# lukashermann/hulc

Measured on AMD Instinct MI355X. Metric: trajectory-windows/sec (seq_len=32, bs=64/GPU), higher is better.
Workload: dtype bf16; 1 GPU; HULC training step, vision goal only (use_clip_auxiliary_loss=false), B=64 windows/GPU, seq_len=32, 200x200 static + 84x84 gripper fp32 NCHW frames, fwd+loss+bwd+Adam, dropout 0.1; global_batch=64, seq_len=32, parallelism=dp1

## Files before the change

### hulc_amd/csrc/engine.h

```cpp
#pragma once
#include <algorithm>
#include <map>
#include <string>
#include <vector>

#include "iengine.h"
#include "gemm.h"
#include "kernels.h"
#include "conv_wgrad.h"
#include "conv_tile.h"
#include "conv_reg.h"
#include "tr_fused.h"
#include "rnn_persist.h"
#include "enc_tail.h"
#include "rollout_step.h"

namespace HULC_NS {

static inline int cdiv(long long a, long long b) { return (int)((a + b - 1) / b); }
#define HIP_CHECK_VOID(x) do { hipError_t e_ = (x); if (e_ != hipSuccess) { hulc_set_error("%s:%d %s", __FILE__, __LINE__, hipGetErrorString(e_)); } } while (0)

template <typename T>
struct Engine : IEngine {
    hulc_config cfg;
// ... 819 lines not shown
    }

    int optim(const hulc_optim& o) override {
        if (!bound) { hulc_set_error("hulc_optimizer_step before hulc_bind_params"); return 1; }
        const bool want_norm = clip_algo == HULC_CLIP_NORM || clip_track;
        if (want_norm && !gn_built) { hulc_set_error("hulc_optimizer_step: the gradient-norm tables are missing (hulc_bind_params / hulc_grad_clip_set build them)"); return 1; }
        persist_check("hulc_optimizer_step", false);
        lazy_sweep(0, numel, st);
        bwd_since_opt = false;
        const unsigned tag = ++opt_seq;
        if (o.kind != HULC_OPT_ADAM && o.kind != HULC_OPT_ADAMW && o.kind != HULC_OPT_SGD) { hulc_set_error("hulc_optimizer_step: unknown optimizer kind %d", (int)o.kind); return 1; }
        if (o.step < 1) { hulc_set_error("hulc_optimizer_step: step counts from 1 (got %lld)", (long long)o.step); return 1; }
        const float lr = o.lr, b1 = o.beta1, b2 = o.beta2, eps = o.eps, gscale = o.grad_scale;
        const int64_t step = o.step;
        const double bc1d = 1.0 - pow((double)b1, (double)step), bc2d = 1.0 - pow((double)b2, (double)step);
        h16_t* const shadow = std::is_same<T, float>::value ? (h16_t*)nullptr : (h16_t*)wshadow;
        const ClipState* const cs = clip_algo != HULC_CLIP_OFF ? clip_state : nullptr;
        if (want_norm) {
            hipLaunchKernelGGL(grad_sumsq_kernel, dim3(gn_chunks), dim3(256), 0, st, (const float*)G, (const long long*)gn_chunk_start, (const int*)gn_chunk_n, gn_partial, scaler);
            hipLaunchKernelGGL(grad_norm_combine_kernel, dim3(1), dim3(1024), 0, st, (const float*)gn_partial, (const int*)gn_tfirst, (int)gn_tens.size(), gscale, (const ScalerState*)scaler,
                               clip_state, gn_tsq, gn_tnorm);
            gn_have = true;
        } else if (scaler) hipLaunchKernelGGL(nonfinite_check_kernel, dim3(2048), dim3(256), 0, st, G, (long long)numel, scaler);
        if (o.kind == HULC_OPT_SGD)
            hipLaunchKernelGGL(sgd_kernel, dim3(2048), dim3(256), 0, st, P, G, AM, (long long)numel, lr, o.momentum, o.dampening, o.weight_decay, (int)(o.nesterov != 0),
                               (int)(step == 1), gscale, shadow, (const ScalerState*)scaler, (const unsigned*)rp_skip, tag, cs);
        else if (adam_fuse_tr && tr_adam.n && shadow) {
            AdamArgs a{P, G, AM, AV, lr, b1, b2, eps, (float)bc1d, (float)sqrt(bc2d), gscale, o.weight_decay, (int)(o.kind == HULC_OPT_ADAMW), shadow, (const ScalerState*)scaler, (const unsigned*)rp_skip, tag, cs};
            hipLaunchKernelGGL(adam_tiled_kernel, dim3(tr_adam.blocks + adam_chunks), dim3(256), 0, st, a, (const TrDesc*)tr_adam.desc, (const unsigned short*)tr_adam.b2d, tr_adam.blocks,
                               (const long long*)adam_chunk_start, (const int*)adam_chunk_n);
            tr_fresh = true;
        } else
            hipLaunchKernelGGL(adam_kernel, dim3(2048), dim3(256), 0, st, P, G, AM, AV, (long long)numel, lr, b1, b2, eps, (float)bc1d, (float)sqrt(bc2d), gscale,
                               shadow, (const ScalerState*)scaler, o.weight_decay, (int)(o.kind == HULC_OPT_ADAMW), (const unsigned*)rp_skip, tag, cs);
        if (scaler) hipLaunchKernelGGL(scaler_update_kernel, dim3(1), dim3(1), 0, st, scaler, (const unsigned*)rp_skip, tag);
        if (hipGetLastError() != hipSuccess) { hulc_set_error("adam launch failed"); return 1; }
        return prepare_weights(true);
    }

    int get_tensor(const char* name, float* out, int64_t cap, int64_t* n) override {
        auto it = named.find(name);
        if (it == named.end()) { hulc_set_error("hulc_get_tensor: unknown tensor '%s'", name); return 1; }
        const Named& t = it->second;
        int64_t cnt = std::min<int64_t>(cap, t.n);
        *n = cnt;
        HIP_CHECK(hipStreamSynchronize(st));
        if (t.kind == 0) { HIP_CHECK(hipMemcpy(out, t.p, cnt * sizeof(float), hipMemcpyDeviceToHost)); }
        else if (t.kind == 1) {
            std::vector<T> tmp(cnt);
            HIP_CHECK(hipMemcpy(tmp.data(), t.p, cnt * sizeof(T), hipMemcpyDeviceToHost));
            for (int64_t i = 0; i < cnt; ++i) out[i] = host_to_f(tmp[i]);
        } else {
            std::vector<int> tmp(cnt);
            HIP_CHECK(hipMemcpy(tmp.data(), t.p, cnt * sizeof(int), hipMemcpyDeviceToHost));
            for (int64_t i = 0; i < cnt; ++i) out[i] = (float)tmp[i];
        }
        return 0;
    }
    static float host_to_f(float x) { return x; }
#ifdef HULC_HALF_F16
    static float host_to_f(h16_t x) {
        const uint32_t sgn = (uint32_t)(x >> 15) << 31, ex = (x >> 10) & 31, man = x & 1023;
        uint32_t u;
        if (ex == 0) { float f = ldexpf((float)man, -24); memcpy(&u, &f, 4); u |= sgn; }
        else if (ex == 31) u = sgn | 0x7f800000u | (man << 13);
        else u = sgn | ((ex + 112) << 23) | (man << 13);
        float f; memcpy(&f, &u, 4); return f;
    }
#else
    static float host_to_f(h16_t x) { uint32_t u = ((uint32_t)x) << 16; float f; memcpy(&f, &u, 4); return f; }
#endif
    int get_plan_idx(int32_t* out, int64_t cap) override {
        HIP_CHECK(hipStreamSynchronize(st));
        int64_t cnt = std::min<int64_t>(cap, (int64_t)cur.B * NCAT);
        HIP_CHECK(hipMemcpy(out, pidx, cnt * sizeof(int), hipMemcpyDeviceToHost));
        return 0;
    }
};

int k_gemm_nt(int is_f32, const void* A, const void* B, float* C, int M, int N, int K, long long lda, long long ldb, long long ldc, const float* bias, int relu,
              void* stream) {
    hipStream_t st = (hipStream_t)stream;
    EpiP ep; ep.out = C; ep.out_f32 = 1; ep.bias = bias; ep.relu = relu & 1;
    if (!is_f32 && !(relu & 4) && M >= 512 && N >= 128) {
        const DenseLoader<h16_t> a = dense<h16_t>((const h16_t*)A, M, lda), b = dense<h16_t>((const h16_t*)B, N, ldb);
        if (gemm_glds_ok(a, b, ep, M, N, K)) {
            launch_gemm_glds(st, a, b, dense_out(ldc), ep, M, N, K);
            if (hipGetLastError() != hipSuccess) { hulc_set_error("hulc_k_gemm_nt: launch failed"); return 1; }
            return 0;
        }
    }
    if (is_f32) {
#ifdef HULC_HALF_F16
        hulc_set_error("hulc_k_gemm_nt: the fp32 kernels live in the bf16 translation unit"); return 1;
#else
        if (M >= 512 && N >= 128) launch_gemm<float, 128, 128>(st, dense<float>((const float*)A, M, lda), dense<float>((const float*)B, N, ldb), dense_out(ldc), ep, M, N, K);
        else launch_gemm<float, 64, 64>(st, dense<float>((const float*)A, M, lda), dense<float>((const float*)B, N, ldb), dense_out(ldc), ep, M, N, K);
#endif
    } else {
        if (M >= 512 && N >= 128) launch_gemm<h16_t, 128, 128>(st, dense<h16_t>((const h16_t*)A, M, lda), dense<h16_t>((const h16_t*)B, N, ldb), dense_out(ldc), ep, M, N, K);
        else launch_gemm<h16_t, 64, 64>(st, dense<h16_t>((const h16_t*)A, M, lda), dense<h16_t>((const h16_t*)B, N, ldb), dense_out(ldc), ep, M, N, K);
    }
    if (hipGetLastError() != hipSuccess) { hulc_set_error("hulc_k_gemm_nt: launch failed"); return 1; }
    return 0;
}

IEngine* make_engine(const hulc_config& cfg, int* rc) {
#ifdef HULC_HALF_F16
    auto* e = new Engine<h16_t>(cfg); *rc = e->alloc_all(); return e;
#else
    if (cfg.dtype == HULC_DTYPE_F32) { auto* e = new Engine<float>(cfg); *rc = e->alloc_all(); return e; }
    auto* e = new Engine<h16_t>(cfg); *rc = e->alloc_all(); return e;
#endif
}

}
```

### hulc_amd/csrc/gemm.h

```cpp
#pragma once
#include "common.h"

namespace HULC_NS {

struct EpiP {
    void* out = nullptr;
    int out_f32 = 0;
    int accumulate = 0;
    int atomic = 0;
    long long z_stride = 0;
    const float* bias = nullptr;
    const float* bias2 = nullptr;
    const void* res = nullptr;
    int res_f32 = 0;
    long long res_ld = 0;
    int res_rowmod = 0;
    int res_late = 0;
    const void* mask = nullptr;
    int mask_tanh = 0;
    int relu = 0;
    float alpha = 1.f;
    float drop_p = 0.f;
    unsigned long long drop_seed = 0;
    void* out2 = nullptr;
// ... 489 lines not shown
        for (int j = 0; j < TN; ++j) acc[i][j] = f32x4{0.f, 0.f, 0.f, 0.f};

    const int wm = wave >> 1, wn = wave & 1;
    if (kbeg < kend) fetch_all(kbeg);
    for (int k = kbeg; k < kend; k += BK) {
#pragma unroll
        for (int i = 0; i < APT; ++i) {
            const int q = tid + i * 256;
            if (q < BM * PPR) tile_commit<T, BM, AL::TRANSPOSED, BK>(As, ra[i], q);
        }
#pragma unroll
        for (int i = 0; i < BPT; ++i) {
            const int q = tid + i * 256;
            if (q < BN * PPR) tile_commit<T, BN, BL::TRANSPOSED, BK>(Bs, rb[i], q);
        }
        __syncthreads();
        if (k + BK < kend) fetch_all(k + BK);
        if constexpr (sizeof(T) == 2) {
            const T* ap = As + (wm * WM + (lane & 15)) * LD + (lane >> 4) * 8;
            const T* bp = Bs + (wn * WN + (lane & 15)) * LD + (lane >> 4) * 8;
#pragma unroll
            for (int kk = 0; kk < BK / 32; ++kk) {
                h16x8_t a[TM], b[TN];
#pragma unroll
                for (int i = 0; i < TM; ++i) a[i] = *reinterpret_cast<const h16x8_t*>(ap + i * 16 * LD + kk * 32);
#pragma unroll
                for (int j = 0; j < TN; ++j) b[j] = *reinterpret_cast<const h16x8_t*>(bp + j * 16 * LD + kk * 32);
#pragma unroll
                for (int i = 0; i < TM; ++i)
#pragma unroll
                    for (int j = 0; j < TN; ++j)
                        acc[i][j] = MFMA_16x16x32_H(b[j], a[i], acc[i][j], 0, 0, 0);
            }
        } else {
            const T* ap = As + (wm * WM + (lane & 15)) * LD + (lane >> 4);
            const T* bp = Bs + (wn * WN + (lane & 15)) * LD + (lane >> 4);
#pragma unroll
            for (int kk = 0; kk < BK / 4; ++kk) {
                float a[TM], b[TN];
#pragma unroll
                for (int i = 0; i < TM; ++i) a[i] = ap[i * 16 * LD + kk * 4];
#pragma unroll
                for (int j = 0; j < TN; ++j) b[j] = bp[j * 16 * LD + kk * 4];
#pragma unroll
                for (int i = 0; i < TM; ++i)
#pragma unroll
                    for (int j = 0; j < TN; ++j)
                        acc[i][j] = __builtin_amdgcn_mfma_f32_16x16x4f32(b[j], a[i], acc[i][j], 0, 0, 0);
            }
        }
        __syncthreads();
    }

    if (tid < BM) rowoff[tid] = (m0 + tid < M) ? om.offset(m0 + tid, zc) : 0;
    __syncthreads();
#pragma unroll
    for (int i = 0; i < TM; ++i) {
        const int row = m0 + wm * WM + i * 16 + (lane & 15);
        if (row < M) {
            const long long obase = rowoff[row - m0] + (long long)zs * ep.z_stride;
            const int rrow = ep.res_rowmod > 0 ? row % ep.res_rowmod : row;
#pragma unroll
            for (int j = 0; j < TN; ++j) {
                const int col = n0 + wn * WN + j * 16 + (lane >> 4) * 4;
                if (col < N) {
                    const float v4[4] = {acc[i][j][0], acc[i][j][1], acc[i][j][2], acc[i][j][3]};
                    epi_store4<T>(ep, v4, rrow, col, N, obase + col);
                }
            }
        }
    }
}

template <typename T, int BM, int BN, typename AL, typename BL, typename OM, int BK = 32>
static inline void launch_gemm(hipStream_t st, const AL& al, const BL& bl, const OM& om, const EpiP& ep, int Mmax, int N,
                               int K, int nclass = 1, int nsplit = 1) {
    if (Mmax <= 0 || N <= 0) return;
    int ksplit = K;
    if (nsplit > 1) ksplit = ((K + nsplit - 1) / nsplit + BK - 1) / BK * BK;
    dim3 grid((Mmax + BM - 1) / BM, (N + BN - 1) / BN, nclass * nsplit);
    hipLaunchKernelGGL((gemm_kernel<T, BM, BN, AL, BL, OM, BK>), grid, dim3(256), 0, st, al, bl, om, ep, N, K, nsplit, ksplit);
}

template <int NST, int NW>
DEVI void gemm_glds_body(const DenseLoader<h16_t>& al, const DenseLoader<h16_t>& bl, const DenseOut& om, const EpiP& ep, int M, int N, int K, int tiles_m, int tiles_n, int bid) {
    constexpr int STAGE = 32 * 1024;
    constexpr int PW = 16 / NW;
    constexpr int TM = 8 / NW * 2 * 2 / 2;
    constexpr int WROWS = TM * 16;
    extern __shared__ __attribute__((aligned(16))) char gg_smem[];
    typedef __attribute__((address_space(3))) char lchar;
    lchar* lds = (lchar*)gg_smem;
    const int tid = threadIdx.x, lane = tid & 63, wave = tid >> 6;
    const int g = lane >> 4, li = lane & 15;
    int tm, tn;
    {
        const int nt = tiles_m * tiles_n, per = nt / 8, rem = nt % 8;
        const int x = bid % 8, q = bid / 8;
        const int tile = x * per + min(x, rem) + q;
        constexpr int GM = 4;
        const int gsz = GM * tiles_n, grp = tile / gsz, first_m = grp * GM, gm = min(GM, tiles_m - first_m);
        tm = first_m + (tile % gsz) % gm;
        tn = (tile % gsz) / gm;
    }
    const int m0 = tm * 128, n0 = tn * 128;
    const int r = lane >> 3, cs = (lane & 7) ^ (r & 6);
    const h16_t* asrc[PW];
    const h16_t* bsrc[PW];
#pragma unroll
    for (int j = 0; j < PW; ++j) {
        asrc[j] = al.row(min(m0 + (wave * PW + j) * 8 + r, M - 1), 0).base + cs * 8;
        bsrc[j] = bl.row(min(n0 + (wave * PW + j) * 8 + r, N - 1), 0).base + cs * 8;
    }
    const int nk = (K + 63) >> 6;
    const bool khalf = (K & 63) != 0;
    auto issue = [&](int kt, int buf) {
        lchar* st = lds + buf * STAGE + wave * PW * 1024;
        long long ko = (long long)kt * 64;
        if (khalf && kt == nk - 1 && cs >= 4) ko -= 32;
#pragma unroll
        for (int j = 0; j < PW; ++j) {
            lds_dma16(asrc[j] + ko, (unsigned)(size_t)(st + j * 1024));
            lds_dma16(bsrc[j] + ko, (unsigned)(size_t)(st + 16384 + j * 1024));
        }
    };
    f32x4 acc[TM][4];
#pragma unroll
    for (int i = 0; i < TM; ++i)
#pragma unroll
        for (int j = 0; j < 4; ++j) acc[i][j] = f32x4{0.f, 0.f, 0.f, 0.f};
    const int wm = wave >> 1, wn = wave & 1;
    const int foff = (li >> 3) * 1024 + (li & 7) * 128;
#pragma unroll
    for (int j = 0; j < NST - 1; ++j)
        if (j < nk) issue(j, j);
    int buf = 0;
#pragma unroll 1
    for (int kt = 0; kt < nk; ++kt) {
        const int ahead = min(NST - 2, nk - 1 - kt);
        if constexpr (PW == 4) {
            if (ahead >= 3) asm volatile("s_waitcnt vmcnt(24)\n\ts_barrier" ::: "memory");
            else if (ahead == 2) asm volatile("s_waitcnt vmcnt(16)\n\ts_barrier" ::: "memory");
            else if (ahead == 1) asm volatile("s_waitcnt vmcnt(8)\n\ts_barrier" ::: "memory");
            else asm volatile("s_waitcnt vmcnt(0)\n\ts_barrier" ::: "memory");
        } else {
            if (ahead >= 3) asm volatile("s_waitcnt vmcnt(12)\n\ts_barrier" ::: "memory");
            else if (ahead == 2) asm volatile("s_waitcnt vmcnt(8)\n\ts_barrier" ::: "memory");
            else if (ahead == 1) asm volatile("s_waitcnt vmcnt(4)\n\ts_barrier" ::: "memory");
            else asm volatile("s_waitcnt vmcnt(0)\n\ts_barrier" ::: "memory");
        }
        if (kt + NST - 1 < nk) issue(kt + NST - 1, buf == 0 ? NST - 1 : buf - 1);
        lchar* sa = lds + buf * STAGE + wm * (WROWS / 8) * 1024 + foff;
        lchar* sb = lds + buf * STAGE + 16384 + wn * 8192 + foff;
        const int nkk = (khalf && kt == nk - 1) ? 1 : 2;
#pragma unroll 1
        for (int kk = 0; kk < nkk; ++kk) {
            const int chunk = (((kk << 2) + g) ^ (li & 6)) << 4;
            h16x8_t a[TM], b[4];
#pragma unroll
            for (int i = 0; i < TM; ++i) a[i] = *(__attribute__((address_space(3))) h16x8_t*)(sa + i * 2048 + chunk);
#pragma unroll
            for (int j = 0; j < 4; ++j) b[j] = *(__attribute__((address_space(3))) h16x8_t*)(sb + j * 2048 + chunk);
#pragma unroll
            for (int i = 0; i < TM; ++i)
#pragma unroll
                for (int j = 0; j < 4; ++j) acc[i][j] = MFMA_16x16x32_H(b[j], a[i], acc[i][j], 0, 0, 0);
        }
        buf = buf == NST - 1 ? 0 : buf + 1;
    }
    const bool plain = epi_is_plain_f32(ep) && (om.s1 & 3) == 0 && (om.s0 & 3) == 0 && ((uintptr_t)ep.out & 15) == 0;
    const bool fast16 = epi_is_fast16(ep) && (om.s1 & 3) == 0 && (om.s0 & 3) == 0;
#pragma unroll
    for (int i = 0; i < TM; ++i) {
        const int row = m0 + wm * WROWS + i * 16 + li;
        if (row < M) {
            const long long obase = om.offset(row, 0);
            const int rrow = ep.res_rowmod > 0 ? row % ep.res_rowmod : row;
#pragma unroll
            for (int j = 0; j < 4; ++j) {
                const int col = n0 + wn * 64 + j * 16 + g * 4;
                if (col < N) {
                    if (plain && col + 3 < N) { epi_plain4(ep, acc[i][j], obase + col); continue; }
                    if (fast16 && col + 3 < N) { epi_fast16_4(ep, acc[i][j], rrow, col, obase + col); continue; }
                    const float v4[4] = {acc[i][j][0], acc[i][j][1], acc[i][j][2], acc[i][j][3]};
                    epi_store4<h16_t>(ep, v4, rrow, col, N, obase + col);
                }
            }
        }
    }
}
template <int NST, int NW>
__global__ void __launch_bounds__(NW * 64) gemm_glds_kernel(DenseLoader<h16_t> al, DenseLoader<h16_t> bl, DenseOut om, EpiP ep, int M, int N, int K,
                                                           int tiles_m, int tiles_n) {
    gemm_glds_body<NST, NW>(al, bl, om, ep, M, N, K, tiles_m, tiles_n, (int)blockIdx.x);
}
struct GemmGroupP { DenseLoader<h16_t> a[3], b[3]; DenseOut om[3]; EpiP ep[3]; int M[3], N[3], K[3], tm[3], tn[3], t0[3]; int n; };
template <int NST, int NW>
__global__ void __launch_bounds__(NW * 64) gemm_glds_group_kernel(GemmGroupP g) {
    const int b = (int)blockIdx.x;
    const int p = (g.n > 2 && b >= g.t0[2]) ? 2 : ((g.n > 1 && b >= g.t0[1]) ? 1 : 0);
    const int bid = b - g.t0[p];
    if (bid >= g.tm[p] * g.tn[p]) return;
    gemm_glds_body<NST, NW>(g.a[p], g.b[p], g.om[p], g.ep[p], g.M[p], g.N[p], g.K[p], g.tm[p], g.tn[p], bid);
}
__global__ void __launch_bounds__(512) gemm_glds_pair_kernel(DenseLoader<h16_t> al, DenseLoader<h16_t> bl1, DenseLoader<h16_t> bl2, DenseOut om, EpiP ep1, EpiP ep2,
                                                           int M, int N, int K, int shs, int tiles_m, int tiles_n) {
    constexpr int NST = 3, NW = 8, STAGE = 48 * 1024, PW = 2, TM = 2, WROWS = 32;
    extern __shared__ __attribute__((aligned(16))) char gg_smem[];
    typedef __attribute__((address_space(3))) char lchar;
    lchar* lds = (lchar*)gg_smem;
    const int tid = threadIdx.x, lane = tid & 63, wave = tid >> 6;
    const int g = lane >> 4, li = lane & 15;
    int tm, tn;
    {
        const int nt = tiles_m * tiles_n, per = nt / 8, rem = nt % 8;
        const int x = blockIdx.x % 8, q = blockIdx.x / 8;
        const int tile = x * per + min(x, rem) + q;
        constexpr int GM = 4;
        const int gsz = GM * tiles_n, grp = tile / gsz, first_m = grp * GM, gm = min(GM, tiles_m - first_m);
        tm = first_m + (tile % gsz) % gm;
        tn = (tile % gsz) / gm;
    }
    const int m0 = tm * 128, n0 = tn * 128;
    const int r = lane >> 3, cs = (lane & 7) ^ (r & 6);
    const h16_t* asrc[PW];
    const h16_t* b1src[PW];
    const h16_t* b2src[PW];
#pragma unroll
    for (int j = 0; j < PW; ++j) {
        asrc[j] = al.row(min(m0 + (wave * PW + j) * 8 + r, M - 1), 0).base + cs * 8;
        b1src[j] = bl1.row(min(n0 + (wave * PW + j) * 8 + r, N - 1), 0).base + cs * 8;
        b2src[j] = bl2.row(min(n0 + (wave * PW + j) * 8 + r, N - 1), 0).base + cs * 8;
    }
    const int nk = K >> 6;
    auto issue = [&](int kt, int buf) {
        lchar* st = lds + buf * STAGE + wave * PW * 1024;
        const long long ko = (long long)kt * 64, ko1 = (long long)max(kt - shs, 0) * 64;
#pragma unroll
        for (int j = 0; j < PW; ++j) {
            lds_dma16(asrc[j] + ko, (unsigned)(size_t)(st + j * 1024));
            lds_dma16(b1src[j] + ko1, (unsigned)(size_t)(st + 16384 + j * 1024));
            lds_dma16(b2src[j] + ko, (unsigned)(size_t)(st + 32768 + j * 1024));
        }
    };
    f32x4 acc1[TM][4], acc2[TM][4];
#pragma unroll
    for (int i = 0; i < TM; ++i)
#pragma unroll
        for (int j = 0; j < 4; ++j) { acc1[i][j] = f32x4{0.f, 0.f, 0.f, 0.f}; acc2[i][j] = f32x4{0.f, 0.f, 0.f, 0.f}; }
    const int wm = wave >> 1, wn = wave & 1;
    const int foff = (li >> 3) * 1024 + (li & 7) * 128;
#pragma unroll
    for (int j = 0; j < NST - 1; ++j)
        if (j < nk) issue(j, j);
    int buf = 0;
#pragma unroll 1
    for (int kt = 0; kt < nk; ++kt) {
        const int ahead = min(NST - 2, nk - 1 - kt);
        if (ahead >= 1) asm volatile("s_waitcnt vmcnt(6)\n\ts_barrier" ::: "memory");
        else asm volatile("s_waitcnt vmcnt(0)\n\ts_barrier" ::: "memory");
        if (kt + NST - 1 < nk) issue(kt + NST - 1, buf == 0 ? NST - 1 : buf - 1);
        lchar* sa = lds + buf * STAGE + wm * (WROWS / 8) * 1024 + foff;
        lchar* sb1 = lds + buf * STAGE + 16384 + wn * 8192 + foff;
        lchar* sb2 = lds + buf * STAGE + 32768 + wn * 8192 + foff;
        const bool with1 = kt >= shs;
#pragma unroll 1
        for (int kk = 0; kk < 2; ++kk) {
            const int chunk = (((kk << 2) + g) ^ (li & 6)) << 4;
            h16x8_t a[TM], b[4], c[4];
#pragma unroll
            for (int i = 0; i < TM; ++i) a[i] = *(__attribute__((address_space(3))) h16x8_t*)(sa + i * 2048 + chunk);
#pragma unroll
            for (int j = 0; j < 4; ++j) b[j] = *(__attribute__((address_space(3))) h16x8_t*)(sb2 + j * 2048 + chunk);
#pragma unroll
            for (int j = 0; j < 4; ++j) c[j] = *(__attribute__((address_space(3))) h16x8_t*)(sb1 + j * 2048 + chunk);
#pragma unroll
            for (int i = 0; i < TM; ++i)
#pragma unroll
                for (int j = 0; j < 4; ++j) acc2[i][j] = MFMA_16x16x32_H(b[j], a[i], acc2[i][j], 0, 0, 0);
            if (with1) {
#pragma unroll
                for (int i = 0; i < TM; ++i)
#pragma unroll
                    for (int j = 0; j < 4; ++j) acc1[i][j] = MFMA_16x16x32_H(c[j], a[i], acc1[i][j], 0, 0, 0);
            }
        }
        buf = buf == NST - 1 ? 0 : buf + 1;
    }
#pragma unroll
    for (int i = 0; i < TM; ++i) {
        const int row = m0 + wm * WROWS + i * 16 + li;
        if (row < M) {
            const long long obase = om.offset(row, 0);
#pragma unroll
            for (int j = 0; j < 4; ++j) {
                const int col = n0 + wn * 64 + j * 16 + g * 4;
                if (col < N) {
                    if (((om.s1 | om.s0) & 3) == 0 && col + 3 < N) { epi_plain4(ep1, acc1[i][j], obase + col); epi_plain4(ep2, acc2[i][j], obase + col); continue; }
                    const float v1[4] = {acc1[i][j][0], acc1[i][j][1], acc1[i][j][2], acc1[i][j][3]};
                    epi_store4<h16_t>(ep1, v1, row, col, N, obase + col);
                    const float v2[4] = {acc2[i][j][0], acc2[i][j][1], acc2[i][j][2], acc2[i][j][3]};
                    epi_store4<h16_t>(ep2, v2, row, col, N, obase + col);
                }
            }
        }
    }
}
static inline bool gemm_glds_pair_ok(const DenseLoader<h16_t>& a, const DenseLoader<h16_t>& b1, const DenseLoader<h16_t>& b2, const EpiP& ep1, const EpiP& ep2, int M, int N, int K, int sh) {
    auto row_ok = [](const DenseLoader<h16_t>& l) { return (l.s0 % 8) == 0 && (l.s1 % 8) == 0 && ((uintptr_t)l.p % 16) == 0 && l.R1 == 0x7fffffff; };
    auto plain = [](const EpiP& e) {
        return !e.generic_only && e.out_f32 && !e.atomic && e.z_stride == 0 && !e.bias && !e.bias2 && !e.res && !e.mask && !e.relu && e.drop_p == 0.f && !e.out2 && e.alpha == 1.f && ((uintptr_t)e.out & 15) == 0;
    };
    return K >= 192 && (K % 64) == 0 && sh > 0 && (sh % 64) == 0 && sh < K && (M % 128) == 0 && (N % 128) == 0 && row_ok(a) && row_ok(b1) && row_ok(b2) && plain(ep1) && plain(ep2);
}
static inline void launch_gemm_glds_pair(hipStream_t st, const DenseLoader<h16_t>& a, const DenseLoader<h16_t>& b1, const DenseLoader<h16_t>& b2, const DenseOut& om, const EpiP& ep1,
                                         const EpiP& ep2, int M, int N, int K, int sh) {
    static bool attr_set = false;
    if (!attr_set) { hipFuncSetAttribute((const void*)gemm_glds_pair_kernel, hipFuncAttributeMaxDynamicSharedMemorySize, 144 * 1024); attr_set = true; }
    const int tiles_m = M / 128, tiles_n = N / 128;
    hipLaunchKernelGGL(gemm_glds_pair_kernel, dim3(tiles_m * tiles_n), dim3(512), 144 * 1024, st, a, b1, b2, om, ep1, ep2, M, N, K, sh / 64, tiles_m, tiles_n);
}
static inline bool gemm_glds_ok(const DenseLoader<h16_t>& a, const DenseLoader<h16_t>& b, const EpiP& ep, int M, int N, int K) {
    auto row_ok = [](const DenseLoader<h16_t>& l) { return (l.s0 % 8) == 0 && (l.s1 % 8) == 0 && ((uintptr_t)l.p % 16) == 0; };
    return K >= 64 && (K % 32) == 0 && ep.z_stride == 0 && row_ok(a) && row_ok(b);
}
static inline void launch_gemm_glds(hipStream_t st, const DenseLoader<h16_t>& a, const DenseLoader<h16_t>& b, const DenseOut& om, const EpiP& ep, int M, int N, int K) {
    static bool attr_set = false;
    if (!attr_set) { hipFuncSetAttribute((const void*)gemm_glds_kernel<3, 8>, hipFuncAttributeMaxDynamicSharedMemorySize, 96 * 1024); attr_set = true; }
    const int tiles_m = (M + 127) / 128, tiles_n = (N + 127) / 128;
    hipLaunchKernelGGL((gemm_glds_kernel<3, 8>), dim3(tiles_m * tiles_n), dim3(512), 96 * 1024, st, a, b, om, ep, M, N, K, tiles_m, tiles_n);
}

static inline void launch_gemm_glds_group(hipStream_t st, GemmGroupP& g) {
    static bool attr_set = false;
    if (!attr_set) { hipFuncSetAttribute((const void*)gemm_glds_group_kernel<3, 8>, hipFuncAttributeMaxDynamicSharedMemorySize, 96 * 1024); attr_set = true; }
    int tot = 0;
    for (int i = 0; i < g.n; ++i) { g.tm[i] = (g.M[i] + 127) / 128; g.tn[i] = (g.N[i] + 127) / 128; g.t0[i] = tot; tot += (g.tm[i] * g.tn[i] + 7) / 8 * 8; }
    hipLaunchKernelGGL((gemm_glds_group_kernel<3, 8>), dim3(tot), dim3(512), 96 * 1024, st, g);
}
template <int NW, int MT, int KS = 0>
__global__ void __launch_bounds__(NW * 64) skinny_gemm_kernel(const h16_t* __restrict__ A, long long lda, const h16_t* __restrict__ W,
                                                             long long ldw, int M, int N, int K, DenseOut om, EpiP ep) {
    __shared__ float red[NW][MT * 256];
    const int tid = threadIdx.x, lane = tid & 63, wave = tid >> 6;
    const int n0 = blockIdx.x * 16;
    const int m0 = blockIdx.y * (MT * 16);
    const int ksteps = K >> 5, kbase = ksteps / NW, krem = ksteps % NW;
    const int kq = KS > 0 ? K / NW : (kbase + (wave < krem ? 1 : 0)) * 32;
    const int kb = KS > 0 ? wave * kq : (wave * kbase + min(wave, krem)) * 32;
    const int g = lane >> 4, i = lane & 15;
    const h16_t* wp = W + (long long)min(n0 + i, N - 1) * ldw + kb + g * 8;
    const h16_t* ap[MT];
#pragma unroll
    for (int mt = 0; mt < MT; ++mt) ap[mt] = A + (long long)min(m0 + mt * 16 + i, M - 1) * lda + kb + g * 8;
    f32x4 acc[MT];
#pragma unroll
    for (int mt = 0; mt < MT; ++mt) acc[mt] = f32x4{0.f, 0.f, 0.f, 0.f};
    if constexpr (KS > 0) {
        h16x8_t b[KS], a[KS][MT];
#pragma unroll
        for (int u = 0; u < KS; ++u) {
            b[u] = *reinterpret_cast<const h16x8_t*>(wp + u * 32);
#pragma unroll
            for (int mt = 0; mt < MT; ++mt) a[u][mt] = *reinterpret_cast<const h16x8_t*>(ap[mt] + u * 32);
        }
#pragma unroll
        for (int u = 0; u < KS; ++u)
#pragma unroll
            for (int mt = 0; mt < MT; ++mt) acc[mt] = MFMA_16x16x32_H(a[u][mt], b[u], acc[mt], 0, 0, 0);
    } else {
    int k = 0;
    for (; k + 128 <= kq; k += 128) {
        h16x8_t b[4], a[4][MT];
#pragma unroll
        for (int u = 0; u < 4; ++u) {
            b[u] = *reinterpret_cast<const h16x8_t*>(wp + k + u * 32);
#pragma unroll
            for (int mt = 0; mt < MT; ++mt) a[u][mt] = *reinterpret_cast<const h16x8_t*>(ap[mt] + k + u * 32);
        }
#pragma unroll
        for (int u = 0; u < 4; ++u)
#pragma unroll
            for (int mt = 0; mt < MT; ++mt) acc[mt] = MFMA_16x16x32_H(a[u][mt], b[u], acc[mt], 0, 0, 0);
    }
    for (; k < kq; k += 32) {
        const h16x8_t b = *reinterpret_cast<const h16x8_t*>(wp + k);
#pragma unroll
        for (int mt = 0; mt < MT; ++mt) {
            const h16x8_t a = *reinterpret_cast<const h16x8_t*>(ap[mt] + k);
            acc[mt] = MFMA_16x16x32_H(a, b, acc[mt], 0, 0, 0);
        }
    }
    }
#pragma unroll
    for (int mt = 0; mt < MT; ++mt)
#pragma unroll
        for (int r = 0; r < 4; ++r) red[wave][(mt * 4 + r) * 64 + lane] = acc[mt][r];
    __syncthreads();
    for (int idx = tid; idx < MT * 256; idx += NW * 64) {
        float v = 0.f;
#pragma unroll
        for (int w = 0; w < NW; ++w) v += red[w][idx];
        const int mt = idx >> 8, r = (idx >> 6) & 3, l = idx & 63;
        const int row = m0 + mt * 16 + (l >> 4) * 4 + r;
        const int col = n0 + (l & 15);
        if (row < M && col < N) {
            const int rrow = ep.res_rowmod > 0 ? row % ep.res_rowmod : row;
            epi_store<h16_t>(ep, v, rrow, col, om.offset(row, 0) + col);
        }
    }
}
#ifdef HULC_KERNEL_STAMPS
__device__ unsigned long long g_stamps[512 * 64];
#define KSTAMP(n) do { if (lane == 0) g_stamps[(blockIdx.y * gridDim.x + blockIdx.x) * 64 + wave * 8 + (n)] = __builtin_amdgcn_s_memtime(); } while (0)
#else
#define KSTAMP(n)
#endif
constexpr int FRAG_PACK_MAX = 24;
struct FragPackBatch { const h16_t* src[FRAG_PACK_MAX]; h16_t* dst[FRAG_PACK_MAX]; int N[FRAG_PACK_MAX], K[FRAG_PACK_MAX]; int blk0[FRAG_PACK_MAX + 1]; int n; };
static inline int frag_pack_blocks(int N, int K) { return (N / 16) * (K / ((K % 256) == 0 ? 256 : 128)); }
__global__ void __launch_bounds__(256) frag_pack_kernel(FragPackBatch b) {
// ... 430 lines not shown
```

Before: 22130 windows/s.

## Split-K across wave halves in LDS-DMA GEMM with register double-buffered fragments

```diff
diff --git a/hulc_amd/csrc/engine.h b/hulc_amd/csrc/engine.h
--- a/hulc_amd/csrc/engine.h
+++ b/hulc_amd/csrc/engine.h
@@ -925,7 +925,7 @@
               void* stream) {
     hipStream_t st = (hipStream_t)stream;
     EpiP ep; ep.out = C; ep.out_f32 = 1; ep.bias = bias; ep.relu = relu & 1;
-    if (!is_f32 && !(relu & 4) && M >= 512 && N >= 128) {
+    if (!is_f32 && !(relu & 4) && ((M >= 512 && N >= 128) || (relu & 8))) {
         const DenseLoader<h16_t> a = dense<h16_t>((const h16_t*)A, M, lda), b = dense<h16_t>((const h16_t*)B, N, ldb);
         if (gemm_glds_ok(a, b, ep, M, N, K)) {
             launch_gemm_glds(st, a, b, dense_out(ldc), ep, M, N, K);
diff --git a/hulc_amd/csrc/gemm.h b/hulc_amd/csrc/gemm.h
--- a/hulc_amd/csrc/gemm.h
+++ b/hulc_amd/csrc/gemm.h
@@ -595,16 +595,17 @@
     hipLaunchKernelGGL((gemm_kernel<T, BM, BN, AL, BL, OM, BK>), grid, dim3(256), 0, st, al, bl, om, ep, N, K, nsplit, ksplit);
 }
 
-template <int NST, int NW>
+template <int NST, bool AHEAD>
 DEVI void gemm_glds_body(const DenseLoader<h16_t>& al, const DenseLoader<h16_t>& bl, const DenseOut& om, const EpiP& ep, int M, int N, int K, int tiles_m, int tiles_n, int bid) {
     constexpr int STAGE = 32 * 1024;
-    constexpr int PW = 16 / NW;
-    constexpr int TM = 8 / NW * 2 * 2 / 2;
-    constexpr int WROWS = TM * 16;
+    constexpr int PW = 2;
+    static_assert(NST * STAGE >= 64 * 1024, "the accumulator exchange uses 64 KB of the ring");
     extern __shared__ __attribute__((aligned(16))) char gg_smem[];
     typedef __attribute__((address_space(3))) char lchar;
+    typedef __attribute__((address_space(3))) h16x8_t lfrag;
+    typedef __attribute__((address_space(3))) f32x4 lf32x4;
     lchar* lds = (lchar*)gg_smem;
-    const int tid = threadIdx.x, lane = tid & 63, wave = tid >> 6;
+    const int tid = threadIdx.x, lane = tid & 63, wave = __builtin_amdgcn_readfirstlane(tid >> 6);
     const int g = lane >> 4, li = lane & 15;
     int tm, tn;
     {
@@ -637,55 +638,120 @@
             lds_dma16(bsrc[j] + ko, (unsigned)(size_t)(st + 16384 + j * 1024));
         }
     };
-    f32x4 acc[TM][4];
-#pragma unroll
-    for (int i = 0; i < TM; ++i)
+    f32x4 acc[4][4];
+#pragma unroll
+    for (int i = 0; i < 4; ++i)
 #pragma unroll
         for (int j = 0; j < 4; ++j) acc[i][j] = f32x4{0.f, 0.f, 0.f, 0.f};
-    const int wm = wave >> 1, wn = wave & 1;
-    const int foff = (li >> 3) * 1024 + (li & 7) * 128;
-#pragma unroll
-    for (int j = 0; j < NST - 1; ++j)
-        if (j < nk) issue(j, j);
-    int buf = 0;
+    const int kh = wave >> 2, wm = (wave >> 1) & 1, wn = wave & 1;
+    const int foff = (li >> 3) * 1024 + (li & 7) * 128 + ((((kh << 2) + g) ^ (li & 6)) << 4);
+    lchar* const fa0 = lds + wm * 8192 + foff;
+    lchar* const fb0 = lds + 16384 + wn * 8192 + foff;
+    const int nmul = nk - ((khalf && kh == 1) ? 1 : 0);
+    auto wait_landed = [&](int ahead) {
+        __builtin_amdgcn_s_waitcnt(0xc07f);
+        if (ahead >= 2) asm volatile("s_waitcnt vmcnt(8)\n\ts_barrier" ::: "memory");
+        else if (ahead == 1) asm volatile("s_waitcnt vmcnt(4)\n\ts_barrier" ::: "memory");
+        else asm volatile("s_waitcnt vmcnt(0)\n\ts_barrier" ::: "memory");
+    };
+    auto read_frags = [&](h16x8_t (&a)[4], h16x8_t (&b)[4], int buf) {
+#pragma unroll
+        for (int i = 0; i < 4; ++i) a[i] = *(lfrag*)(fa0 + buf * STAGE + i * 2048);
+#pragma unroll
+        for (int j = 0; j < 4; ++j) b[j] = *(lfrag*)(fb0 + buf * STAGE + j * 2048);
+    };
+    auto multiply = [&](const h16x8_t (&a)[4], const h16x8_t (&b)[4]) {
+#pragma unroll
+        for (int i = 0; i < 4; ++i)
+#pragma unroll
+            for (int j = 0; j < 4; ++j) acc[i][j] = MFMA_16x16x32_H(b[j], a[i], acc[i][j], 0, 0, 0);
+    };
+    if constexpr (AHEAD) {
+        static_assert(NST == 3, "the waits below count at most two stages in flight behind the awaited one");
+#pragma unroll
+        for (int j = 0; j < NST; ++j)
+            if (j < nk) issue(j, j);
+        h16x8_t a0[4], b0[4], a1[4], b1[4];
+        wait_landed(min(NST, nk) - 1);
+        read_frags(a0, b0, 0);
+        int buf = 0;
+        auto step = [&](int kt, const h16x8_t (&ca)[4], const h16x8_t (&cb)[4], h16x8_t (&na)[4], h16x8_t (&nb)[4]) {
+            if (kt + 1 < nk) {
+                wait_landed(min(NST - 2, nk - 2 - kt));
+                if (kt + NST < nk) issue(kt + NST, buf);
+                buf = buf == NST - 1 ? 0 : buf + 1;
+                read_frags(na, nb, buf);
+            }
+            if (kt < nmul) multiply(ca, cb);
+        };
+        auto steady = [&](int kt, const h16x8_t (&ca)[4], const h16x8_t (&cb)[4], h16x8_t (&na)[4], h16x8_t (&nb)[4]) {
+            __builtin_amdgcn_s_waitcnt(0xc07f);
+            asm volatile("s_waitcnt vmcnt(4)\n\ts_barrier" ::: "memory");
+            issue(kt + NST, buf);
+            buf = buf == NST - 1 ? 0 : buf + 1;
+            read_frags(na, nb, buf);
+            multiply(ca, cb);
+#pragma unroll
+            for (int q = 0; q < 8; ++q) {
+                __builtin_amdgcn_sched_group_barrier(0x100, 1, 0);
+                __builtin_amdgcn_sched_group_barrier(0x008, 2, 0);
+            }
+        };
+        int kt = 0;
 #pragma unroll 1
-    for (int kt = 0; kt < nk; ++kt) {
-        const int ahead = min(NST - 2, nk - 1 - kt);
-        if constexpr (PW == 4) {
-            if (ahead >= 3) asm volatile("s_waitcnt vmcnt(24)\n\ts_barrier" ::: "memory");
-            else if (ahead == 2) asm volatile("s_waitcnt vmcnt(16)\n\ts_barrier" ::: "memory");
-            else if (ahead == 1) asm volatile("s_waitcnt vmcnt(8)\n\ts_barrier" ::: "memory");
-            else asm volatile("s_waitcnt vmcnt(0)\n\ts_barrier" ::: "memory");
+        for (; kt + NST + 1 < nk; kt += 2) {
+            steady(kt, a0, b0, a1, b1);
+            steady(kt + 1, a1, b1, a0, b0);
+        }
+#pragma unroll 1
+        for (; kt < nk; kt += 2) {
+            step(kt, a0, b0, a1, b1);
+            if (kt + 1 < nk) step(kt + 1, a1, b1, a0, b0);
+        }
+    } else {
+#pragma unroll
+        for (int j = 0; j < NST - 1; ++j)
+            if (j < nk) issue(j, j);
+        int buf = 0;
+#pragma unroll 1
+        for (int kt = 0; kt < nk; ++kt) {
+            wait_landed(min(NST - 2, nk - 1 - kt));
+            if (kt + NST - 1 < nk) issue(kt + NST - 1, buf == 0 ? NST - 1 : buf - 1);
+            if (kt < nmul) {
+                h16x8_t a[4], b[4];
+                read_frags(a, b, buf);
+                multiply(a, b);
+            }
+            buf = buf == NST - 1 ? 0 : buf + 1;
+        }
+    }
+    f32x4 mine[2][4];
+    {
+        lf32x4* const xw = (lf32x4*)(lds + (wave & 3) * 16384 + kh * 8192) + lane;
+        lf32x4* const xr = (lf32x4*)(lds + (wave & 3) * 16384 + (kh ^ 1) * 8192) + lane;
+        __syncthreads();
+        if (kh == 0) {
+#pragma unroll
+            for (int i = 0; i < 2; ++i)
+#pragma unroll
+                for (int j = 0; j < 4; ++j) { xw[(i * 4 + j) * 64] = acc[2 + i][j]; mine[i][j] = acc[i][j]; }
         } else {
-            if (ahead >= 3) asm volatile("s_waitcnt vmcnt(12)\n\ts_barrier" ::: "memory");
-            else if (ahead == 2) asm volatile("s_waitcnt vmcnt(8)\n\ts_barrier" ::: "memory");
-            else if (ahead == 1) asm volatile("s_waitcnt vmcnt(4)\n\ts_barrier" ::: "memory");
-            else asm volatile("s_waitcnt vmcnt(0)\n\ts_barrier" ::: "memory");
-        }
-        if (kt + NST - 1 < nk) issue(kt + NST - 1, buf == 0 ? NST - 1 : buf - 1);
-        lchar* sa = lds + buf * STAGE + wm * (WROWS / 8) * 1024 + foff;
-        lchar* sb = lds + buf * STAGE + 16384 + wn * 8192 + foff;
-        const int nkk = (khalf && kt == nk - 1) ? 1 : 2;
-#pragma unroll 1
-        for (int kk = 0; kk < nkk; ++kk) {
-            const int chunk = (((kk << 2) + g) ^ (li & 6)) << 4;
-            h16x8_t a[TM], b[4];
-#pragma unroll
-            for (int i = 0; i < TM; ++i) a[i] = *(__attribute__((address_space(3))) h16x8_t*)(sa + i * 2048 + chunk);
-#pragma unroll
-            for (int j = 0; j < 4; ++j) b[j] = *(__attribute__((address_space(3))) h16x8_t*)(sb + j * 2048 + chunk);
-#pragma unroll
-            for (int i = 0; i < TM; ++i)
-#pragma unroll
-                for (int j = 0; j < 4; ++j) acc[i][j] = MFMA_16x16x32_H(b[j], a[i], acc[i][j], 0, 0, 0);
-        }
-        buf = buf == NST - 1 ? 0 : buf + 1;
+#pragma unroll
+            for (int i = 0; i < 2; ++i)
+#pragma unroll
+                for (int j = 0; j < 4; ++j) { xw[(i * 4 + j) * 64] = acc[i][j]; mine[i][j] = acc[2 + i][j]; }
+        }
+        __syncthreads();
+#pragma unroll
+        for (int i = 0; i < 2; ++i)
+#pragma unroll
+            for (int j = 0; j < 4; ++j) mine[i][j] += xr[(i * 4 + j) * 64];
     }
     const bool plain = epi_is_plain_f32(ep) && (om.s1 & 3) == 0 && (om.s0 & 3) == 0 && ((uintptr_t)ep.out & 15) == 0;
     const bool fast16 = epi_is_fast16(ep) && (om.s1 & 3) == 0 && (om.s0 & 3) == 0;
 #pragma unroll
-    for (int i = 0; i < TM; ++i) {
-        const int row = m0 + wm * WROWS + i * 16 + li;
+    for (int i = 0; i < 2; ++i) {
+        const int row = m0 + wm * 64 + kh * 32 + i * 16 + li;
         if (row < M) {
             const long long obase = om.offset(row, 0);
             const int rrow = ep.res_rowmod > 0 ? row % ep.res_rowmod : row;
@@ -693,36 +759,37 @@
             for (int j = 0; j < 4; ++j) {
                 const int col = n0 + wn * 64 + j * 16 + g * 4;
                 if (col < N) {
-                    if (plain && col + 3 < N) { epi_plain4(ep, acc[i][j], obase + col); continue; }
-                    if (fast16 && col + 3 < N) { epi_fast16_4(ep, acc[i][j], rrow, col, obase + col); continue; }
-                    const float v4[4] = {acc[i][j][0], acc[i][j][1], acc[i][j][2], acc[i][j][3]};
+                    if (plain && col + 3 < N) { epi_plain4(ep, mine[i][j], obase + col); continue; }
+                    if (fast16 && col + 3 < N) { epi_fast16_4(ep, mine[i][j], rrow, col, obase + col); continue; }
+                    const float v4[4] = {mine[i][j][0], mine[i][j][1], mine[i][j][2], mine[i][j][3]};
                     epi_store4<h16_t>(ep, v4, rrow, col, N, obase + col);
                 }
             }
         }
     }
 }
-template <int NST, int NW>
-__global__ void __launch_bounds__(NW * 64) gemm_glds_kernel(DenseLoader<h16_t> al, DenseLoader<h16_t> bl, DenseOut om, EpiP ep, int M, int N, int K,
-                                                           int tiles_m, int tiles_n) {
-    gemm_glds_body<NST, NW>(al, bl, om, ep, M, N, K, tiles_m, tiles_n, (int)blockIdx.x);
+template <int NST, bool AHEAD>
+__global__ void __launch_bounds__(512) gemm_glds_kernel(DenseLoader<h16_t> al, DenseLoader<h16_t> bl, DenseOut om, EpiP ep, int M, int N, int K,
+                                                        int tiles_m, int tiles_n) {
+    gemm_glds_body<NST, AHEAD>(al, bl, om, ep, M, N, K, tiles_m, tiles_n, (int)blockIdx.x);
 }
 struct GemmGroupP { DenseLoader<h16_t> a[3], b[3]; DenseOut om[3]; EpiP ep[3]; int M[3], N[3], K[3], tm[3], tn[3], t0[3]; int n; };
-template <int NST, int NW>
-__global__ void __launch_bounds__(NW * 64) gemm_glds_group_kernel(GemmGroupP g) {
+template <int NST, bool AHEAD>
+__global__ void __launch_bounds__(512) gemm_glds_group_kernel(GemmGroupP g) {
     const int b = (int)blockIdx.x;
     const int p = (g.n > 2 && b >= g.t0[2]) ? 2 : ((g.n > 1 && b >= g.t0[1]) ? 1 : 0);
     const int bid = b - g.t0[p];
     if (bid >= g.tm[p] * g.tn[p]) return;
-    gemm_glds_body<NST, NW>(g.a[p], g.b[p], g.om[p], g.ep[p], g.M[p], g.N[p], g.K[p], g.tm[p], g.tn[p], bid);
+    gemm_glds_body<NST, AHEAD>(g.a[p], g.b[p], g.om[p], g.ep[p], g.M[p], g.N[p], g.K[p], g.tm[p], g.tn[p], bid);
 }
 __global__ void __launch_bounds__(512) gemm_glds_pair_kernel(DenseLoader<h16_t> al, DenseLoader<h16_t> bl1, DenseLoader<h16_t> bl2, DenseOut om, EpiP ep1, EpiP ep2,
                                                            int M, int N, int K, int shs, int tiles_m, int tiles_n) {
-    constexpr int NST = 3, NW = 8, STAGE = 48 * 1024, PW = 2, TM = 2, WROWS = 32;
+    constexpr int NST = 3, STAGE = 48 * 1024, PW = 2;
     extern __shared__ __attribute__((aligned(16))) char gg_smem[];
     typedef __attribute__((address_space(3))) char lchar;
+    typedef __attribute__((address_space(3))) f32x4 lf32x4;
     lchar* lds = (lchar*)gg_smem;
-    const int tid = threadIdx.x, lane = tid & 63, wave = tid >> 6;
+    const int tid = threadIdx.x, lane = tid & 63, wave = __builtin_amdgcn_readfirstlane(tid >> 6);
     const int g = lane >> 4, li = lane & 15;
     int tm, tn;
     {
@@ -756,13 +823,13 @@
             lds_dma16(b2src[j] + ko, (unsigned)(size_t)(st + 32768 + j * 1024));
         }
     };
-    f32x4 acc1[TM][4], acc2[TM][4];
-#pragma unroll
-    for (int i = 0; i < TM; ++i)
+    f32x4 acc1[4][4], acc2[4][4];
+#pragma unroll
+    for (int i = 0; i < 4; ++i)
 #pragma unroll
         for (int j = 0; j < 4; ++j) { acc1[i][j] = f32x4{0.f, 0.f, 0.f, 0.f}; acc2[i][j] = f32x4{0.f, 0.f, 0.f, 0.f}; }
-    const int wm = wave >> 1, wn = wave & 1;
-    const int foff = (li >> 3) * 1024 + (li & 7) * 128;
+    const int kh = wave >> 2, wm = (wave >> 1) & 1, wn = wave & 1;
+    const int foff = (li >> 3) * 1024 + (li & 7) * 128 + ((((kh << 2) + g) ^ (li & 6)) << 4);
 #pragma unroll
     for (int j = 0; j < NST - 1; ++j)
         if (j < nk) issue(j, j);
@@ -773,36 +840,51 @@
         if (ahead >= 1) asm volatile("s_waitcnt vmcnt(6)\n\ts_barrier" ::: "memory");
         else asm volatile("s_waitcnt vmcnt(0)\n\ts_barrier" ::: "memory");
         if (kt + NST - 1 < nk) issue(kt + NST - 1, buf == 0 ? NST - 1 : buf - 1);
-        lchar* sa = lds + buf * STAGE + wm * (WROWS / 8) * 1024 + foff;
+        lchar* sa = lds + buf * STAGE + wm * 8192 + foff;
         lchar* sb1 = lds + buf * STAGE + 16384 + wn * 8192 + foff;
         lchar* sb2 = lds + buf * STAGE + 32768 + wn * 8192 + foff;
         const bool with1 = kt >= shs;
-#pragma unroll 1
-        for (int kk = 0; kk < 2; ++kk) {
-            const int chunk = (((kk << 2) + g) ^ (li & 6)) << 4;
-            h16x8_t a[TM], b[4], c[4];
-#pragma unroll
-            for (int i = 0; i < TM; ++i) a[i] = *(__attribute__((address_space(3))) h16x8_t*)(sa + i * 2048 + chunk);
-#pragma unroll
-            for (int j = 0; j < 4; ++j) b[j] = *(__attribute__((address_space(3))) h16x8_t*)(sb2 + j * 2048 + chunk);
-#pragma unroll
-            for (int j = 0; j < 4; ++j) c[j] = *(__attribute__((address_space(3))) h16x8_t*)(sb1 + j * 2048 + chunk);
-#pragma unroll
-            for (int i = 0; i < TM; ++i)
+        {
+            h16x8_t a[4], b[4], c[4];
+#pragma unroll
+            for (int i = 0; i < 4; ++i) a[i] = *(__attribute__((address_space(3))) h16x8_t*)(sa + i * 2048);
+#pragma unroll
+            for (int j = 0; j < 4; ++j) b[j] = *(__attribute__((address_space(3))) h16x8_t*)(sb2 + j * 2048);
+#pragma unroll
+            for (int j = 0; j < 4; ++j) c[j] = *(__attribute__((address_space(3))) h16x8_t*)(sb1 + j * 2048);
+#pragma unroll
+            for (int i = 0; i < 4; ++i)
 #pragma unroll
                 for (int j = 0; j < 4; ++j) acc2[i][j] = MFMA_16x16x32_H(b[j], a[i], acc2[i][j], 0, 0, 0);
             if (with1) {
 #pragma unroll
-                for (int i = 0; i < TM; ++i)
+                for (int i = 0; i < 4; ++i)
 #pragma unroll
                     for (int j = 0; j < 4; ++j) acc1[i][j] = MFMA_16x16x32_H(c[j], a[i], acc1[i][j], 0, 0, 0);
             }
         }
         buf = buf == NST - 1 ? 0 : buf + 1;
     }
-#pragma unroll
-    for (int i = 0; i < TM; ++i) {
-        const int row = m0 + wm * WROWS + i * 16 + li;
+    {
+        lf32x4* const xw = (lf32x4*)(lds + (wave & 3) * 32768 + kh * 16384) + lane;
+        lf32x4* const xr = (lf32x4*)(lds + (wave & 3) * 32768 + (kh ^ 1) * 16384) + lane;
+        __syncthreads();
+#pragma unroll
+        for (int i = 0; i < 2; ++i)
+#pragma unroll
+            for (int j = 0; j < 4; ++j) {
+                if (kh == 0) { xw[(i * 4 + j) * 64] = acc1[2 + i][j]; xw[(8 + i * 4 + j) * 64] = acc2[2 + i][j]; }
+                else { xw[(i * 4 + j) * 64] = acc1[i][j]; xw[(8 + i * 4 + j) * 64] = acc2[i][j]; acc1[i][j] = acc1[2 + i][j]; acc2[i][j] = acc2[2 + i][j]; }
+            }
+        __syncthreads();
+#pragma unroll
+        for (int i = 0; i < 2; ++i)
+#pragma unroll
+            for (int j = 0; j < 4; ++j) { acc1[i][j] += xr[(i * 4 + j) * 64]; acc2[i][j] += xr[(8 + i * 4 + j) * 64]; }
+    }
+#pragma unroll
+    for (int i = 0; i < 2; ++i) {
+        const int row = m0 + wm * 64 + kh * 32 + i * 16 + li;
         if (row < M) {
             const long long obase = om.offset(row, 0);
 #pragma unroll
@@ -839,17 +921,17 @@
 }
 static inline void launch_gemm_glds(hipStream_t st, const DenseLoader<h16_t>& a, const DenseLoader<h16_t>& b, const DenseOut& om, const EpiP& ep, int M, int N, int K) {
     static bool attr_set = false;
-    if (!attr_set) { hipFuncSetAttribute((const void*)gemm_glds_kernel<3, 8>, hipFuncAttributeMaxDynamicSharedMemorySize, 96 * 1024); attr_set = true; }
+    if (!attr_set) { hipFuncSetAttribute((const void*)gemm_glds_kernel<3, true>, hipFuncAttributeMaxDynamicSharedMemorySize, 96 * 1024); attr_set = true; }
     const int tiles_m = (M + 127) / 128, tiles_n = (N + 127) / 128;
-    hipLaunchKernelGGL((gemm_glds_kernel<3, 8>), dim3(tiles_m * tiles_n), dim3(512), 96 * 1024, st, a, b, om, ep, M, N, K, tiles_m, tiles_n);
+    hipLaunchKernelGGL((gemm_glds_kernel<3, true>), dim3(tiles_m * tiles_n), dim3(512), 96 * 1024, st, a, b, om, ep, M, N, K, tiles_m, tiles_n);
 }
 
 static inline void launch_gemm_glds_group(hipStream_t st, GemmGroupP& g) {
     static bool attr_set = false;
-    if (!attr_set) { hipFuncSetAttribute((const void*)gemm_glds_group_kernel<3, 8>, hipFuncAttributeMaxDynamicSharedMemorySize, 96 * 1024); attr_set = true; }
+    if (!attr_set) { hipFuncSetAttribute((const void*)gemm_glds_group_kernel<3, true>, hipFuncAttributeMaxDynamicSharedMemorySize, 96 * 1024); attr_set = true; }
     int tot = 0;
     for (int i = 0; i < g.n; ++i) { g.tm[i] = (g.M[i] + 127) / 128; g.tn[i] = (g.N[i] + 127) / 128; g.t0[i] = tot; tot += (g.tm[i] * g.tn[i] + 7) / 8 * 8; }
-    hipLaunchKernelGGL((gemm_glds_group_kernel<3, 8>), dim3(tot), dim3(512), 96 * 1024, st, g);
+    hipLaunchKernelGGL((gemm_glds_group_kernel<3, true>), dim3(tot), dim3(512), 96 * 1024, st, g);
 }
 template <int NW, int MT, int KS = 0>
 __global__ void __launch_bounds__(NW * 64) skinny_gemm_kernel(const h16_t* __restrict__ A, long long lda, const h16_t* __restrict__ W,
```

New measurement: 22240 windows/s, median of 6. Within noise of the previous version (+0.5%).
